# Sirui-Xu/InterDiff

Measured on AMD Instinct MI355X. Metric: denoising frame-steps/sec (denoising-steps/sec x B x T frames), higher is better.
Workload: dtype f32 (every contraction of the denoiser -- feed-forward block, QKV projection, self-attention, row-block contractions and the two token GEMMs: every fp32 operand as two f16 planes, 3 f16 MFMAs per product, fp32 accumulate; SMPL and everything else fp32 MFMA / VALU)

## Files before the change

### interdiff_amd/csrc/gemm.h

```cpp
#pragma once
#include "common.h"
#include "philox.h"

namespace idf_gemm {

enum { A_PLAIN = 0, A_LN = 1, A_TOKT = 2, A_TOKT_R = 3 };
constexpr bool is_tokt(int a) { return a == A_TOKT || a == A_TOKT_R; }
enum { E_BIAS = 0, E_GELU = 1, E_RESID = 2, E_HEADS = 3, E_EMBED = 4, E_HEADS_POST = 5, E_HEADS_POST_RAGGED = 6,
       E_SKEL = 7, E_SKEL_POST = 8, E_SKEL_POST_RAGGED = 9 };
constexpr bool is_skel(int epi) { return epi == E_SKEL || epi == E_SKEL_POST || epi == E_SKEL_POST_RAGGED; }
constexpr bool is_post(int epi) { return epi == E_HEADS_POST || epi == E_HEADS_POST_RAGGED || epi == E_SKEL_POST || epi == E_SKEL_POST_RAGGED; }

struct Args {
    const float *A;
    int lda, K;
    int Ka;
    const float *lnw, *lnb;
    size_t a_pstride;
    const float *W;
    const float *bias;
    float *C;
    int ldc, M, N;
    float *xn_out;
    const float *resid;
    int T;
    const int64_t *ts;
    const float *temb, *pe;
    int n_steps;
    float *post_x;
    const float *post_gt;
    const uint8_t *post_mask;
    const float *post_table;
    const int64_t *post_state;
#ifdef IDF_GEMM_PROBE
    long long *probe;
#endif
};

__device__ __forceinline__ void xcd_tile(int ntn, int &mt, int &nt, int &wg) {
    const int nwg = gridDim.x, id = blockIdx.x, q = nwg >> 3, r = nwg & 7, xcd = id & 7;
    wg = (xcd < r ? xcd * (q + 1) : r * (q + 1) + (xcd - r) * q) + (id >> 3);
    mt = wg / ntn;
    nt = wg - mt * ntn;
}

__device__ __forceinline__ float4 ld4(const float *p) { return *reinterpret_cast<const float4 *>(p); }
__device__ __forceinline__ float4 zero4() { return make_float4(0.f, 0.f, 0.f, 0.f); }

#ifdef IDF_GEMM_PROBE
#define IDF_PROBE_STAMP(g, wg, slot) do { if ((g).probe && threadIdx.x == 0) (g).probe[(wg) * 4 + (slot)] = clock64(); } while (0)
#else
#define IDF_PROBE_STAMP(g, wg, slot) do { } while (0)
#endif

#define IDF_MFMA4(acc, a, b)                                            \
    do {                                                                \
        acc = __builtin_amdgcn_mfma_f32_16x16x4f32(a, b, acc, 0, 0, 0); \
    } while (0)


template <int TN>
__device__ __forceinline__ void load_bias(const Args &g, float (&bv)[TN], int col0) {
#pragma unroll
    for (int j = 0; j < TN; ++j) bv[j] = g.bias ? g.bias[min(col0 + j * 16, g.N - 1)] : 0.f;
}

template <int TM, int TN>
__device__ __forceinline__ void load_resid(const Args &g, float (&rres)[TM][TN][4], int rbase0, int col0) {
#pragma unroll
    for (int i = 0; i < TM; ++i)
#pragma unroll
        for (int j = 0; j < TN; ++j) {
            const int col = min(col0 + j * 16, g.N - 1);
#pragma unroll
            for (int r = 0; r < 4; ++r) rres[i][j][r] = g.resid[(size_t)min(rbase0 + i * 16 + r, g.M - 1) * g.ldc + col];
        }
}

template <int TM, int TN>
__device__ __forceinline__ void load_embed_add(const Args &g, float (&rres)[TM][TN][4], int rbase0, int col0) {
#pragma unroll
    for (int i = 0; i < TM; ++i)
#pragma unroll
        for (int r = 0; r < 4; ++r) {
            const int rc = min(rbase0 + i * 16 + r, g.M - 1), b = rc / g.T, t = rc - b * g.T;
            int64_t step = g.ts[b];
            step = step < 0 ? 0 : (step >= g.n_steps ? g.n_steps - 1 : step);
#pragma unroll
            for (int j = 0; j < TN; ++j) {
                const int cc = min(col0 + j * 16, g.N - 1);
                rres[i][j][r] = g.temb[(size_t)step * g.N + cc] + g.pe[(size_t)t * g.N + cc];
            }
        }
}

template <int TM, int TN>
struct PostOperands {
    float4 xv[TM][TN], gv[TM][TN], e[TM][TN];
    uchar4 mk[TM][TN];
    float c1, c2, sigma;
};
__device__ __forceinline__ float sel8(const float4 a, const float4 b, int k) {
    const float lo = k == 0 ? a.x : (k == 1 ? a.y : (k == 2 ? a.z : a.w));
    const float hi = k == 4 ? b.x : (k == 5 ? b.y : (k == 6 ? b.z : b.w));
    return k < 4 ? lo : hi;
}
template <int TM, int TN, bool ragged>
__device__ __forceinline__ void post_prefetch(const Args &g, PostOperands<TM, TN> &po, int rbase0, int col0) {
    const int64_t st = g.post_state[4];
    const uint64_t it = (uint64_t)g.post_state[5], seed = (uint64_t)g.post_state[2];
    const size_t elem0 = (size_t)g.post_state[6];
    po.c1 = g.post_table[st * 4]; po.c2 = g.post_table[st * 4 + 1]; po.sigma = g.post_table[st * 4 + 2];
#pragma unroll
    for (int i = 0; i < TM; ++i)
#pragma unroll
        for (int j = 0; j < TN; ++j) {
            const int col = min(col0 + j * 16, g.N - 1);
            if constexpr (!ragged) {
                const int rbase = min(rbase0 + i * 16, g.M - 4);
                const int b = rbase / g.T, t = rbase - b * g.T;
                const size_t flat = ((size_t)b * g.N + col) * g.T + t;
                po.xv[i][j] = ld4(g.post_x + flat);
                po.gv[i][j] = g.post_mask ? ld4(g.post_gt + flat) : zero4();
                po.mk[i][j] = g.post_mask ? *reinterpret_cast<const uchar4 *>(g.post_mask + flat) : make_uchar4(0, 0, 0, 0);
                po.e[i][j] = randn4(seed, it, (uint64_t)((flat + elem0) >> 2));
            } else {
                const int r0 = min(rbase0 + i * 16, g.M - 1), b0 = r0 / g.T;
                const size_t idx0 = ((size_t)b0 * g.N + col) * g.T + (r0 - b0 * g.T) + elem0;
                const float4 ea = randn4(seed, it, (uint64_t)(idx0 >> 2)), eb = randn4(seed, it, (uint64_t)(idx0 >> 2) + 1);
                float xr[4], gr[4], er[4];
                unsigned char mr[4];
#pragma unroll
                for (int r = 0; r < 4; ++r) {
                    const int row = min(rbase0 + i * 16 + r, g.M - 1), b = row / g.T;
                    const size_t flat = ((size_t)b * g.N + col) * g.T + (row - b * g.T);
                    xr[r] = g.post_x[flat];
                    gr[r] = g.post_mask ? g.post_gt[flat] : 0.f;
                    mr[r] = g.post_mask ? g.post_mask[flat] : (unsigned char)0;
                    if (b == b0) er[r] = sel8(ea, eb, (int)(idx0 & 3) + (row - r0));
                    else {
                        const size_t idx = flat + elem0;
                        const float4 ec = randn4(seed, it, (uint64_t)(idx >> 2));
                        er[r] = sel8(ec, ec, (int)(idx & 3));
                    }
                }
                po.xv[i][j] = make_float4(xr[0], xr[1], xr[2], xr[3]);
                po.gv[i][j] = make_float4(gr[0], gr[1], gr[2], gr[3]);
                po.mk[i][j] = make_uchar4(mr[0], mr[1], mr[2], mr[3]);
                po.e[i][j] = make_float4(er[0], er[1], er[2], er[3]);
            }
            asm volatile("" : "+v"(po.e[i][j].x), "+v"(po.e[i][j].y), "+v"(po.e[i][j].z), "+v"(po.e[i][j].w));
        }
}
template <int TM, int TN, bool ragged>
__device__ __forceinline__ void epilogue_post(const Args &g, const f32x4 (&acc)[TM][TN], const float (&bvs)[TN], const PostOperands<TM, TN> &po,
                                              int rbase0, int col0, float *lds_tile = nullptr, int lds_stride = 0) {
#pragma unroll
    for (int i = 0; i < TM; ++i)
#pragma unroll
        for (int j = 0; j < TN; ++j) {
            const int rbase = rbase0 + i * 16, col = col0 + j * 16;
            if (col >= g.N || rbase >= g.M) continue;
            const float bv = bvs[j];
            float4 pv = make_float4(acc[i][j][0] + bv, acc[i][j][1] + bv, acc[i][j][2] + bv, acc[i][j][3] + bv);
            const uchar4 m = po.mk[i][j];
            const float4 gv = po.gv[i][j];
            pv.x = m.x ? gv.x : pv.x; pv.y = m.y ? gv.y : pv.y; pv.z = m.z ? gv.z : pv.z; pv.w = m.w ? gv.w : pv.w;
            const float4 out = posterior4(po.c1, po.c2, po.sigma, pv, po.xv[i][j], po.e[i][j]);
            if (lds_tile) {
                lds_tile[0] = out.x; lds_tile[lds_stride] = out.y; lds_tile[2 * lds_stride] = out.z; lds_tile[3 * lds_stride] = out.w;
            }
            if constexpr (!ragged) {
                const int b = rbase / g.T, t = rbase - b * g.T;
                idf_store16_wt(g.post_x + ((size_t)b * g.N + col) * g.T + t, out);
            } else {
                const float ov[4] = {out.x, out.y, out.z, out.w};
#pragma unroll
                for (int r = 0; r < 4; ++r) {
                    const int row = rbase + r, b = row / g.T;
                    if (row < g.M) idf_store4_wt(g.post_x + ((size_t)b * g.N + col) * g.T + (row - b * g.T), ov[r]);
                }
            }
        }
}

template <int TM, int TN, int EPI>
__device__ __forceinline__ void epilogue(const Args &g, const f32x4 (&acc)[TM][TN], const float (&rres)[TM][TN][4],
                                         const float (&bvs)[TN], int rbase0, int col0) {
    const int M = g.M, N = g.N;
#pragma unroll
    for (int i = 0; i < TM; ++i) {
        const int rbase = rbase0 + i * 16;
#pragma unroll
        for (int j = 0; j < TN; ++j) {
            const int col = col0 + j * 16;
            const bool colok = col < N;
            const float bv = bvs[j];
            if constexpr (EPI == E_HEADS) {
                if (!colok) continue;
                const int b = rbase / g.T, t = rbase - b * g.T;
                if ((g.T & 3) == 0 && rbase + 3 < M) {
                    *reinterpret_cast<float4 *>(g.C + ((size_t)b * N + col) * g.T + t) =
                        make_float4(acc[i][j][0] + bv, acc[i][j][1] + bv, acc[i][j][2] + bv, acc[i][j][3] + bv);
                } else {
#pragma unroll
                    for (int r = 0; r < 4; ++r) {
                        const int row = rbase + r;
                        if (row >= M) continue;
                        const int bb = row / g.T, tt = row - bb * g.T;
                        g.C[((size_t)bb * N + col) * g.T + tt] = acc[i][j][r] + bv;
                    }
                }
            } else {
#pragma unroll
                for (int r = 0; r < 4; ++r) {
                    const int row = rbase + r;
                    float v = acc[i][j][r] + bv;
                    if constexpr (EPI == E_GELU) v = gelu_fast(v);
                    if constexpr (EPI == E_RESID) v += rres[i][j][r];
                    if constexpr (EPI == E_EMBED) {
                        const int rc = min(row, M - 1), b = rc / g.T, t = rc - b * g.T, cc = min(col, N - 1);
                        int64_t step = g.ts[b];
                        step = step < 0 ? 0 : (step >= g.n_steps ? g.n_steps - 1 : step);
                        v += g.temb[(size_t)step * N + cc] + g.pe[(size_t)t * N + cc];
                    }
                    if (row < M && colok) g.C[(size_t)row * g.ldc + col] = v;
                }
            }
        }
    }
}

template <int BM, int BN, int TM, int TN, int EPI, int NT>
__device__ __forceinline__ void epilogue_rows(const Args &g, float *cs, const f32x4 (&acc)[TM][TN], const float (&rres)[TM][TN][4],
                                              const float (&bvs)[TN], bool writer, int wrow0, int wcol0, int kq, int li, int m0, int n0,
                                              int tid) {
    constexpr int CS = BN + 4, Q = BN / 4;
    if (writer) {
#pragma unroll
        for (int i = 0; i < TM; ++i)
#pragma unroll
            for (int j = 0; j < TN; ++j)
#pragma unroll
                for (int r = 0; r < 4; ++r) {
                    float v = acc[i][j][r] + bvs[j];
                    if constexpr (EPI == E_GELU) v = gelu_fast(v);
                    if constexpr (EPI == E_RESID || EPI == E_EMBED) v += rres[i][j][r];
                    cs[(wrow0 + i * 16 + kq * 4 + r) * CS + wcol0 + j * 16 + li] = v;
                }
    }
    __syncthreads();
    for (int idx = tid; idx < BM * Q; idx += NT) {
        const int row = idx / Q, c4 = idx - row * Q, gr = m0 + row, gc = n0 + c4 * 4;
        if (gr < g.M && gc < g.N) idf_store16_wt(g.C + (size_t)gr * g.ldc + gc, ld4(cs + row * CS + c4 * 4));
    }
}

}
#include "skel_head.h"
namespace idf_gemm {

template <int BM, int BN, int WM, int WN, int KC, int APRO, int EPI, int NP = 1>
__global__ __launch_bounds__(WM *WN * 64) void gemm_kernel(const Args g) {
    constexpr int NT = WM * WN * 64;
    constexpr int TM = BM / WM / 16, TN = BN / WN / 16;
    constexpr int QC = KC / 4;
    constexpr int AQ = BM * 4 + 4, BQ = BN * 4 + 4;
    constexpr int KLN = 256;
    constexpr int A_FLOATS = APRO == A_LN ? (KLN / 4) * AQ : 2 * QC * AQ;
    constexpr int LA = (BM * QC + NT - 1) / NT, LB = (BN * QC + NT - 1) / NT;
    static_assert(TM >= 1 && TN >= 1 && QC % 4 == 0, "tile shape");
    __shared__ __attribute__((aligned(16))) float smem[A_FLOATS + 2 * QC * BQ];
    float *As = smem, *Bs = smem + A_FLOATS;

    idf_args_now(g.A, g.lda, g.K, g.lnw, g.lnb, g.a_pstride, g.W, g.bias, g.C, g.ldc, g.M, g.N, g.xn_out, g.resid, g.T, g.ts, g.temb, g.pe, g.n_steps,
                 g.post_x, g.post_gt, g.post_mask, g.post_table, g.post_state, gridDim.x);
    const int tid = threadIdx.x, lane = tid & 63, wave = tid >> 6;
    int mt_, nt_, wg;
    xcd_tile((g.N + BN - 1) / BN, mt_, nt_, wg);
    const int m0 = mt_ * BM, n0 = nt_ * BN;
    const int wm = wave / WN, wn = wave % WN;
    const int li = lane & 15, kq = lane >> 4;
    const int K = g.K, M = g.M, N = g.N;
    const int nk = (K + KC - 1) / KC;

    float4 areg[LA], breg[LB];
    auto load_b = [&](int kc) {
#pragma unroll
        for (int i = 0; i < LB; ++i) {
            const int f = tid + NT * i;
            if ((BN * QC) % NT == 0 || f < BN * QC) {
                const int col = f / QC, q = f % QC, n = n0 + col, k = kc * KC + q * 4;
                breg[i] = (n < N && k < K) ? ld4(g.W + (size_t)n * K + k) : zero4();
            }
        }
    };
    auto store_b = [&](int buf) {
#pragma unroll
        for (int i = 0; i < LB; ++i) {
            const int f = tid + NT * i;
            if ((BN * QC) % NT == 0 || f < BN * QC) {
                const int col = f / QC, q = f % QC;
                *reinterpret_cast<float4 *>(Bs + (buf * QC + q) * BQ + col * 4) = breg[i];
            }
        }
    };
    auto load_a = [&](int kc) {
#pragma unroll
        for (int i = 0; i < LA; ++i) {
            const int f = tid + NT * i;
            if ((BM * QC) % NT == 0 || f < BM * QC) {
                if constexpr (APRO == A_TOKT) {
                    const int row = f % BM, q = f / BM, m = m0 + row, k = kc * KC + q * 4;
                    float4 v = zero4();
                    if (m < M && k < K) {
                        const int b = m / g.T, t = m - b * g.T;
                        const float *p = g.A + ((size_t)b * K + k) * g.T + t;
                        v.x = p[0];
                        v.y = p[(size_t)g.T];
                        v.z = p[(size_t)2 * g.T];
                        v.w = p[(size_t)3 * g.T];
                    }
                    areg[i] = v;
                } else if constexpr (APRO == A_TOKT_R) {
                    const int row = f % BM, q = f / BM, m = m0 + row, k = kc * KC + q * 4, Ka = g.Ka;
                    float4 v = zero4();
                    if (m < M && k < Ka) {
                        const int b = m / g.T, t = m - b * g.T;
                        const float *p = g.A + ((size_t)b * Ka + k) * g.T + t;
                        const float y = p[(size_t)min(1, Ka - 1 - k) * g.T], z = p[(size_t)min(2, Ka - 1 - k) * g.T], w_ = p[(size_t)min(3, Ka - 1 - k) * g.T];
                        v.x = p[0];
                        v.y = k + 1 < Ka ? y : 0.f;
                        v.z = k + 2 < Ka ? z : 0.f;
                        v.w = k + 3 < Ka ? w_ : 0.f;
                    }
                    areg[i] = v;
                } else {
                    const int row = f / QC, q = f % QC, m = m0 + row, k = kc * KC + q * 4;
                    areg[i] = (m < M && k < K) ? ld4(g.A + (size_t)m * g.lda + k) : zero4();
                }
            }
        }
    };
    auto store_a = [&](int buf) {
#pragma unroll
        for (int i = 0; i < LA; ++i) {
            const int f = tid + NT * i;
            if ((BM * QC) % NT == 0 || f < BM * QC) {
                const int row = is_tokt(APRO) ? f % BM : f / QC, q = is_tokt(APRO) ? f / BM : f % QC;
                *reinterpret_cast<float4 *>(As + (buf * QC + q) * AQ + row * 4) = areg[i];
            }
        }
    };

    IDF_PROBE_STAMP(g, wg, 0);
    load_b(0);
    float rres[TM][TN][4], bvs[TN];
    load_bias<TN>(g, bvs, n0 + wn * TN * 16 + li);
    if constexpr (EPI == E_RESID) load_resid<TM, TN>(g, rres, m0 + wm * TM * 16 + kq * 4, n0 + wn * TN * 16 + li);
    if constexpr (EPI == E_EMBED) load_embed_add<TM, TN>(g, rres, m0 + wm * TM * 16 + kq * 4, n0 + wn * TN * 16 + li);
    if constexpr (APRO == A_LN) {
        constexpr int NW = WM * WN;
        const float4 gw = g.lnw ? ld4(g.lnw + lane * 4) : make_float4(1.f, 1.f, 1.f, 1.f);
        const float4 gb = g.lnw ? ld4(g.lnb + lane * 4) : zero4();
#pragma unroll
        for (int i = 0; i < BM / NW; ++i) {
            const int row = wave + NW * i, m = m0 + row;
            float4 v = ld4_sum<NP>(g.A + (size_t)min(m, M - 1) * g.lda + lane * 4, g.a_pstride);
            if (g.lnw) {
                float mean, rstd;
                ln_row_stats(v, mean, rstd);
                v.x = (v.x - mean) * rstd * gw.x + gb.x;
                v.y = (v.y - mean) * rstd * gw.y + gb.y;
                v.z = (v.z - mean) * rstd * gw.z + gb.z;
                v.w = (v.w - mean) * rstd * gw.w + gb.w;
            }
            *reinterpret_cast<float4 *>(As + lane * AQ + row * 4) = v;
            if (g.xn_out && nt_ == 0 && m < M) *reinterpret_cast<float4 *>(g.xn_out + (size_t)m * KLN + lane * 4) = v;
        }
    } else {
        load_a(0);
        store_a(0);
    }
    store_b(0);
    __syncthreads();
    IDF_PROBE_STAMP(g, wg, 1);

    f32x4 acc[TM][TN];
#pragma unroll
    for (int i = 0; i < TM; ++i)
#pragma unroll
        for (int j = 0; j < TN; ++j) acc[i][j] = f32x4{0.f, 0.f, 0.f, 0.f};

    for (int kc = 0; kc < nk; ++kc) {
        const int buf = kc & 1;
        if (kc + 1 < nk) {
            load_b(kc + 1);
            if constexpr (APRO != A_LN) load_a(kc + 1);
        }
        const float *Ab = APRO == A_LN ? As + kc * QC * AQ : As + buf * QC * AQ;
        const float *Bb = Bs + buf * QC * BQ;
#pragma unroll
        for (int s = 0; s < QC / 4; ++s) {
            float4 a[TM], b[TN];
#pragma unroll
            for (int i = 0; i < TM; ++i) a[i] = ld4(Ab + (s * 4 + kq) * AQ + ((wm * TM + i) * 16 + li) * 4);
#pragma unroll
            for (int j = 0; j < TN; ++j) b[j] = ld4(Bb + (s * 4 + kq) * BQ + ((wn * TN + j) * 16 + li) * 4);
#pragma unroll
            for (int i = 0; i < TM; ++i)
#pragma unroll
                for (int j = 0; j < TN; ++j) IDF_MFMA4(acc[i][j], a[i].x, b[j].x);
#pragma unroll
            for (int i = 0; i < TM; ++i)
#pragma unroll
                for (int j = 0; j < TN; ++j) IDF_MFMA4(acc[i][j], a[i].y, b[j].y);
#pragma unroll
            for (int i = 0; i < TM; ++i)
#pragma unroll
                for (int j = 0; j < TN; ++j) IDF_MFMA4(acc[i][j], a[i].z, b[j].z);
#pragma unroll
            for (int i = 0; i < TM; ++i)
#pragma unroll
                for (int j = 0; j < TN; ++j) IDF_MFMA4(acc[i][j], a[i].w, b[j].w);
        }
        if (kc + 1 < nk) {
            store_b(buf ^ 1);
            if constexpr (APRO != A_LN) store_a(buf ^ 1);
        }
        __syncthreads();
    }

    IDF_PROBE_STAMP(g, wg, 2);
    if constexpr (EPI == E_BIAS || EPI == E_GELU || EPI == E_RESID || EPI == E_EMBED) {
        static_assert(BM * (BN + 4) <= A_FLOATS + 2 * QC * BQ, "C tile must fit the operand buffers");
        epilogue_rows<BM, BN, TM, TN, EPI, NT>(g, smem, acc, rres, bvs, true, wm * TM * 16, wn * TN * 16, kq, li, m0, n0, tid);
    } else {
        epilogue<TM, TN, EPI>(g, acc, rres, bvs, m0 + wm * TM * 16 + kq * 4, n0 + wn * TN * 16 + li);
    }
    IDF_PROBE_STAMP(g, wg, 3);
}

template <int BM, int BN, int WM, int WN, int KC, int APRO, int EPI, int NP = 1>
inline void launch(hipStream_t s, const Args &g) {
    dim3 grid((unsigned)(idf_cdiv(g.M, BM) * idf_cdiv(g.N, BN)));
    hipLaunchKernelGGL((gemm_kernel<BM, BN, WM, WN, KC, APRO, EPI, NP>), grid, dim3(WM * WN * 64), 0, s, g);
}

template <int N>
__device__ __forceinline__ void wait_vmcnt() {
    static_assert(N >= 0 && N <= 16, "vmcnt literal");
#define IDF_VMCNT_CASE(n) if constexpr (N == n) asm volatile("s_waitcnt vmcnt(" #n ")" ::: "memory");
    IDF_VMCNT_CASE(0) IDF_VMCNT_CASE(1) IDF_VMCNT_CASE(2) IDF_VMCNT_CASE(3) IDF_VMCNT_CASE(4) IDF_VMCNT_CASE(5) IDF_VMCNT_CASE(6)
    IDF_VMCNT_CASE(7) IDF_VMCNT_CASE(8) IDF_VMCNT_CASE(9) IDF_VMCNT_CASE(10) IDF_VMCNT_CASE(11) IDF_VMCNT_CASE(12)
    IDF_VMCNT_CASE(13) IDF_VMCNT_CASE(14) IDF_VMCNT_CASE(15) IDF_VMCNT_CASE(16)
#undef IDF_VMCNT_CASE
}

template <int BM, int BN, int WM, int WN, int KS, int KC, int APRO, int EPI, int NS = 3, int NP = 1>
__global__ __launch_bounds__(WM *WN *KS * 64) void gemm_glds_kernel(const Args g) {
    constexpr int NWT = WM * WN, NW = NWT * KS;
    constexpr int TM = BM / WM / 16, TN = BN / WN / 16;
    constexpr int CH = KC / 4;
    constexpr int RSL = 256 + 4;
    constexpr int A_STAGE = APRO == A_LN ? 0 : BM * KC, STAGE = A_STAGE + BN * KC;
    constexpr int A_LN_FLOATS = APRO == A_LN ? BM * RSL : 0;
    constexpr int IA = A_STAGE / 256, IB = BN * KC / 256, IPC = IA + IB, LPC = IPC / NW;
    constexpr int RED = KS > 1 ? (KS - 1) * NWT * 64 * TM * TN * 4 : 0;
    static_assert(IPC % NW == 0 && LPC >= 1 && (NS - 2) * LPC <= 16 && NS >= 3 && NS <= 6, "chunk loads must split evenly over the waves");
    static_assert((CH / 4) % KS == 0 && TM >= 1 && TN >= 1 && (CH == 8 || CH == 16), "tile shape");
    static_assert(APRO != A_TOKT, "token gather uses the register-staged kernel");
    constexpr int SMEM = A_LN_FLOATS + NS * STAGE;
    __shared__ __attribute__((aligned(1024))) float smem[SMEM > RED ? SMEM : RED];
    float *Aln = smem, *stages = smem + A_LN_FLOATS;

    idf_args_now(g.A, g.lda, g.K, g.lnw, g.lnb, g.a_pstride, g.W, g.bias, g.C, g.ldc, g.M, g.N, g.xn_out, g.resid, g.T, g.ts, g.temb, g.pe, g.n_steps,
                 g.post_x, g.post_gt, g.post_mask, g.post_table, g.post_state, gridDim.x);
    const int tid = threadIdx.x, lane = tid & 63;
    const int wave = __builtin_amdgcn_readfirstlane(tid >> 6);
    int mt_, nt_, wg;
    xcd_tile((g.N + BN - 1) / BN, mt_, nt_, wg);
    const int m0 = mt_ * BM, n0 = nt_ * BN;
    const int ks = wave / NWT, wt = wave % NWT, wm = wt / WN, wn = wt % WN;
    const int li = lane & 15, kq = lane >> 4;
    const int K = g.K, M = g.M, N = g.N;
    const int nk = K / KC;
    IDF_PROBE_STAMP(g, wg, 0);

    const float *src[LPC];
    int dst[LPC];
#pragma unroll
    for (int j = 0; j < LPC; ++j) {
        const int i = wave + NW * j;
        if (i < IA) {
            const int p = i * 64 + lane, row = p / CH, c = (p % CH) ^ (row % CH);
            src[j] = g.A + (size_t)min(m0 + row, M - 1) * g.lda + c * 4;
            dst[j] = i * 256;
        } else {
            const int ib = i - IA, p = ib * 64 + lane, row = p / CH, c = (p % CH) ^ (row % CH);
            src[j] = g.W + (size_t)min(n0 + row, N - 1) * K + c * 4;
            dst[j] = A_STAGE + ib * 256;
        }
    }
    auto wait_landed = [&](int c) {
        const int ahead = min(NS - 2, nk - 1 - c);
        if (ahead <= 0) wait_vmcnt<0>();
        else if (ahead == 1) wait_vmcnt<LPC>();
        else if (ahead == 2) { if constexpr (NS >= 4) wait_vmcnt<2 * LPC>(); }
        else if (ahead == 3) { if constexpr (NS >= 5) wait_vmcnt<3 * LPC>(); }
        else { if constexpr (NS >= 6) wait_vmcnt<4 * LPC>(); }
    };
    const uint32_t stages_lds = idf_lds_addr(stages);
    auto issue = [&](int kc, int st) {
#pragma unroll
        for (int j = 0; j < LPC; ++j) idf_dma16_v(src[j] + kc * KC, stages_lds + (uint32_t)((st * STAGE + dst[j]) * 4));
    };

#pragma unroll
    for (int c = 0; c < NS - 1; ++c)
        if (c < nk) issue(c, c);
    float rres[TM][TN][4], bvs[TN];
    load_bias<TN>(g, bvs, n0 + wn * TN * 16 + li);
    if constexpr (EPI == E_RESID) {
        if (ks == 0) load_resid<TM, TN>(g, rres, m0 + wm * TM * 16 + kq * 4, n0 + wn * TN * 16 + li);
    }
    PostOperands<is_post(EPI) && !is_skel(EPI) ? TM : 1, is_post(EPI) && !is_skel(EPI) ? TN : 1> po;
    SkelPre skp;
    if constexpr (is_skel(EPI)) {
        static_assert(!is_skel(EPI) || (BM == 32 && BN == 32 && NW == 8 && SMEM >= 32 * SKH_CS + 32 * SKH_ZMAX), "the keypoint head's tile: 32 x 32, 512 threads");
        skel_prefetch<EPI>(g, skp, m0, nt_, tid);
    } else if constexpr (is_post(EPI)) {
        if (ks == 0) post_prefetch<TM, TN, EPI == E_HEADS_POST_RAGGED>(g, po, m0 + wm * TM * 16 + kq * 4, n0 + wn * TN * 16 + li);
    }
    if constexpr (APRO == A_LN) {
        const float4 gw = g.lnw ? ld4(g.lnw + lane * 4) : make_float4(1.f, 1.f, 1.f, 1.f);
        const float4 gb = g.lnw ? ld4(g.lnb + lane * 4) : zero4();
#pragma unroll
        for (int i = 0; i < BM / NW; ++i) {
            const int row = wave + NW * i, m = m0 + row;
            float4 v = ld4_sum<NP>(g.A + (size_t)min(m, M - 1) * g.lda + lane * 4, g.a_pstride);
            if (g.lnw) {
                float mean, rstd;
                ln_row_stats(v, mean, rstd);
                v.x = (v.x - mean) * rstd * gw.x + gb.x;
                v.y = (v.y - mean) * rstd * gw.y + gb.y;
                v.z = (v.z - mean) * rstd * gw.z + gb.z;
                v.w = (v.w - mean) * rstd * gw.w + gb.w;
            }
            *reinterpret_cast<float4 *>(Aln + row * RSL + lane * 4) = v;
            if (g.xn_out && nt_ == 0 && m < M) *reinterpret_cast<float4 *>(g.xn_out + (size_t)m * 256 + lane * 4) = v;
        }
    }
    wait_landed(0);
    __builtin_amdgcn_s_waitcnt(0xc07f);
    __builtin_amdgcn_s_barrier();
    IDF_PROBE_STAMP(g, wg, 1);

    f32x4 acc[TM][TN];
#pragma unroll
    for (int i = 0; i < TM; ++i)
#pragma unroll
        for (int j = 0; j < TN; ++j) acc[i][j] = f32x4{0.f, 0.f, 0.f, 0.f};

    int aoff[TM], akey[TM], boff[TN], bkey[TN];
#pragma unroll
    for (int i = 0; i < TM; ++i) {
        const int row = (wm * TM + i) * 16 + li;
        aoff[i] = APRO == A_LN ? row * RSL : row * KC;
        akey[i] = row % CH;
    }
#pragma unroll
    for (int j = 0; j < TN; ++j) {
        const int row = (wn * TN + j) * 16 + li;
        boff[j] = row * KC;
        bkey[j] = row % CH;
    }

    int st = 0;
    for (int kc = 0; kc < nk; ++kc) {
        if (kc + NS - 1 < nk) issue(kc + NS - 1, st >= 1 ? st - 1 : NS - 1);
        const float *Ab = APRO == A_LN ? Aln + kc * KC : stages + st * STAGE;
        const float *Bb = stages + st * STAGE + A_STAGE;
#pragma unroll
        for (int s2 = 0; s2 < CH / 4 / KS; ++s2) {
            const int c = (s2 * KS + ks) * 4 + kq;
            float4 a[TM], b[TN];
#pragma unroll
            for (int i = 0; i < TM; ++i) a[i] = ld4(Ab + aoff[i] + (APRO == A_LN ? c : (c ^ akey[i])) * 4);
#pragma unroll
            for (int j = 0; j < TN; ++j) b[j] = ld4(Bb + boff[j] + (c ^ bkey[j]) * 4);
#pragma unroll
            for (int i = 0; i < TM; ++i)
#pragma unroll
                for (int j = 0; j < TN; ++j) IDF_MFMA4(acc[i][j], a[i].x, b[j].x);
#pragma unroll
            for (int i = 0; i < TM; ++i)
#pragma unroll
                for (int j = 0; j < TN; ++j) IDF_MFMA4(acc[i][j], a[i].y, b[j].y);
#pragma unroll
            for (int i = 0; i < TM; ++i)
#pragma unroll
                for (int j = 0; j < TN; ++j) IDF_MFMA4(acc[i][j], a[i].z, b[j].z);
#pragma unroll
            for (int i = 0; i < TM; ++i)
#pragma unroll
                for (int j = 0; j < TN; ++j) IDF_MFMA4(acc[i][j], a[i].w, b[j].w);
        }
        wait_landed(kc + 1);
        __builtin_amdgcn_s_waitcnt(0xc07f);
        __builtin_amdgcn_s_barrier();
        st = st == NS - 1 ? 0 : st + 1;
    }
    IDF_PROBE_STAMP(g, wg, 2);

    if constexpr (KS > 1) {
        constexpr int SLAB = NWT * 64 * TM * TN * 4;
        float *red = smem + (size_t)(wt * 64 + lane) * (TM * TN * 4);
        if (ks > 0) {
#pragma unroll
            for (int i = 0; i < TM; ++i)
#pragma unroll
                for (int j = 0; j < TN; ++j) *reinterpret_cast<f32x4 *>(red + (ks - 1) * SLAB + (i * TN + j) * 4) = acc[i][j];
        }
        __syncthreads();
        if (ks == 0) {
#pragma unroll
            for (int q = 0; q < KS - 1; ++q)
#pragma unroll
                for (int i = 0; i < TM; ++i)
#pragma unroll
                    for (int j = 0; j < TN; ++j) acc[i][j] += *reinterpret_cast<const f32x4 *>(red + q * SLAB + (i * TN + j) * 4);
        }
    }
    if constexpr (EPI == E_BIAS || EPI == E_GELU || EPI == E_RESID) {
        static_assert(BM * (BN + 4) <= (SMEM > RED ? SMEM : RED), "C tile must fit the operand buffers");
        if constexpr (KS > 1) __syncthreads();
        epilogue_rows<BM, BN, TM, TN, EPI, NW * 64>(g, smem, acc, rres, bvs, ks == 0, wm * TM * 16, wn * TN * 16, kq, li, m0, n0, tid);
    } else if constexpr (is_skel(EPI)) {
        __syncthreads();
        if (ks == 0) {
#pragma unroll
            for (int i = 0; i < TM; ++i)
#pragma unroll
                for (int j = 0; j < TN; ++j)
#pragma unroll
                    for (int r = 0; r < 4; ++r) smem[((wm * TM + i) * 16 + kq * 4 + r) * SKH_CS + (wn * TN + j) * 16 + li] = acc[i][j][r] + bvs[j];
        }
        skel_epilogue<EPI>(g, smem, smem + 32 * SKH_CS, skp, m0, nt_, tid);
    } else {
        if constexpr (is_post(EPI)) {
            if (ks == 0) epilogue_post<TM, TN, EPI == E_HEADS_POST_RAGGED>(g, acc, bvs, po, m0 + wm * TM * 16 + kq * 4, n0 + wn * TN * 16 + li);
        } else {
            if (ks == 0) epilogue<TM, TN, EPI>(g, acc, rres, bvs, m0 + wm * TM * 16 + kq * 4, n0 + wn * TN * 16 + li);
        }
    }
    IDF_PROBE_STAMP(g, wg, 3);
}

template <int BM, int BN, int WM, int WN, int KS, int KC, int APRO, int EPI, int NS = 3, int NP = 1>
inline void launch_glds(hipStream_t s, const Args &g) {
    dim3 grid((unsigned)(idf_cdiv(g.M, BM) * idf_cdiv(g.N, BN)));
    hipLaunchKernelGGL((gemm_glds_kernel<BM, BN, WM, WN, KS, KC, APRO, EPI, NS, NP>), grid, dim3(WM * WN * KS * 64), 0, s, g);
}

}
```

### interdiff_amd/csrc/tail_h2.h

```cpp
#pragma once
#include "common.h"
#include "gemm.h"
#include "ffn_h2.h"

namespace idf_tail_h2 {

using idf_ffn_h2::h8;
constexpr int D = IDF_MDM_D, CW = 144, TRW = 16, NTH = 512, NWV = NTH / 64;
constexpr int NTO = CW / 16, KSH = D / 32;
constexpr int KE = 160, KSE = KE / 32, NTE = D / 16;
constexpr int OUT_H2_FLOATS = NTO * KSH * 2 * 64 * 4, IN_H2_FLOATS = NTE * KSE * 2 * 64 * 4;
constexpr int RHS = D + 8;
constexpr int XTS = CW + 4;
constexpr int XHS = KE + 8;
constexpr int USS = D + 4;

struct TailArgs {
    const float *u_in;
    size_t pstride;
    const float *ln_w, *ln_b;
    const float *wout, *out_b;
    float *x0;
    idf_gemm::Args post;
    const float *x_tok;
    const float *win, *in_b, *temb, *pe;
    const int64_t *ts;
    int n_steps;
    float *u0;
    int M, T;
    int plain_ids;
};

template <int MODE, bool RAGGED>
__global__ __launch_bounds__(NTH) void step_tail_h2_kernel(const float *__restrict__ u_in, size_t u_pstride, const float *__restrict__ wout, int M, int T, int nwg,
                                                           int plain_ids, const TailArgs a) {
    constexpr bool HEADS = MODE != 0, EMBED = MODE == 0 || MODE == 3, POST = MODE >= 2;
    asm volatile("" ::: "v255");
    __shared__ __attribute__((aligned(16))) _Float16 rpl[HEADS ? 2 * TRW * RHS : 8];
    __shared__ __attribute__((aligned(16))) float xt[EMBED ? TRW * XTS : 4];
    __shared__ __attribute__((aligned(16))) _Float16 xpl[EMBED ? 2 * TRW * XHS : 8];
    __shared__ float sc[TRW];
    __shared__ __attribute__((aligned(16))) float us[EMBED ? TRW * USS : 4];
    const int tid = threadIdx.x, lane = tid & 63, wave = tid >> 6, li = lane & 15, kq = lane >> 4;
    const int wid = blockIdx.x, xq = nwg >> 3, xr = nwg & 7, xcd = wid & 7;
    const int tile = plain_ids ? wid : (xcd < xr ? xcd * (xq + 1) : xr * (xq + 1) + (xcd - xr) * xq) + (wid >> 3);
    const int m0 = tile * TRW;
    const int rown = (wave & 3) * 4 + kq;
    const bool rowpass = wave < 4;

    if constexpr (HEADS) {
        constexpr int NTW = 2;
        const int ntw = wave == 0 ? 2 : 1;
        auto tile_of = [&](int j) { return j == 0 ? wave : NTO - 1; };
        Row16Raw<IDF_FFN_SLICES> raw;
        if (rowpass) raw.request(u_in + (size_t)min(m0 + rown, M - 1) * D, li, u_pstride);
        idf_gemm::PostOperands<1, 1> po[NTW];
        if constexpr (POST) {
#pragma unroll
            for (int j = 0; j < NTW; ++j)
                if (j < ntw) idf_gemm::post_prefetch<1, 1, RAGGED>(a.post, po[j], m0 + kq * 4, tile_of(j) * 16 + li);
        }
        float4 wf[NTW][KSH][2];
#pragma unroll
        for (int j = 0; j < NTW; ++j)
            if (j < ntw) {
#pragma unroll
                for (int s = 0; s < KSH; ++s)
#pragma unroll
                    for (int pl = 0; pl < 2; ++pl) wf[j][s][pl] = idf_gemm::ld4(wout + (size_t)(((tile_of(j) * KSH + s) * 2 + pl) * 64 + lane) * 4);
            }
        if (rowpass) {
            Row16 r;
            raw.reduce(r);
            ln_row16(r, a.ln_w, a.ln_b, li);
            idf_ffn_h2::row16_store_planes(r, rpl + rown * RHS, rpl + (TRW + rown) * RHS, li);
        }
        __syncthreads();
        f32x4 am[NTW], ac[NTW];
#pragma unroll
        for (int j = 0; j < NTW; ++j) am[j] = ac[j] = f32x4{0.f, 0.f, 0.f, 0.f};
        h8 ah[KSH], al[KSH];
#pragma unroll
        for (int s = 0; s < KSH; ++s) {
            ah[s] = *reinterpret_cast<const h8 *>(rpl + li * RHS + 32 * s + 8 * kq);
            al[s] = *reinterpret_cast<const h8 *>(rpl + (TRW + li) * RHS + 32 * s + 8 * kq);
        }
#pragma unroll
        for (int j = 0; j < NTW; ++j)
            if (j < ntw) {
#pragma unroll
                for (int s = 0; s < KSH; ++s) {
                    IDF_H2_MFMA(am[j], ah[s], __builtin_bit_cast(h8, wf[j][s][0]));
                    IDF_H2_MFMA(ac[j], ah[s], __builtin_bit_cast(h8, wf[j][s][1]));
                    IDF_H2_MFMA(ac[j], al[s], __builtin_bit_cast(h8, wf[j][s][0]));
                }
            }
#pragma unroll
        for (int j = 0; j < NTW; ++j)
            if (j < ntw) {
                const int col = tile_of(j) * 16 + li, rbase = m0 + kq * 4;
                const float bv = a.out_b[col];
                f32x4 v;
#pragma unroll
                for (int q = 0; q < 4; ++q) v[q] = am[j][q] + ac[j][q] * idf_ffn_h2::LO_UNSCALE;
                if constexpr (POST) {
                    const f32x4 accs[1][1] = {{v}};
                    const float bvs[1] = {bv};
                    idf_gemm::epilogue_post<1, 1, RAGGED>(a.post, accs, bvs, po[j], rbase, col, EMBED ? xt + (kq * 4) * XTS + col : nullptr, XTS);
                } else {
                    if (!RAGGED && rbase + 3 < M) {
                        const int b = rbase / T, t = rbase - b * T;
                        *reinterpret_cast<float4 *>(a.x0 + ((size_t)b * CW + col) * T + t) = make_float4(v[0] + bv, v[1] + bv, v[2] + bv, v[3] + bv);
                    } else {
#pragma unroll
                        for (int q = 0; q < 4; ++q) {
                            const int row = rbase + q;
                            if (row < M) {
                                const int bb = row / T;
                                a.x0[((size_t)bb * CW + col) * T + (row - bb * T)] = v[q] + bv;
                            }
                        }
                    }
                }
            }
    }

    if constexpr (EMBED) {
        if constexpr (MODE == 0) {
            if constexpr (!RAGGED) {
#pragma unroll
                for (int it = 0; it < (CW * 4 + NTH - 1) / NTH; ++it) {
                    const int idx = tid + it * NTH, c = min(idx >> 2, CW - 1), rg = idx & 3;
                    const int rowb = min(m0 + 4 * rg, M - 4), b = rowb / T, t = rowb - b * T;
                    const float4 v = idf_gemm::ld4(a.x_tok + ((size_t)b * CW + c) * T + t);
                    if (idx < CW * 4) {
                        float *d = xt + (4 * rg) * XTS + c;
                        d[0] = v.x; d[XTS] = v.y; d[2 * XTS] = v.z; d[3 * XTS] = v.w;
                    }
                }
            } else {
#pragma unroll
                for (int it = 0; it < (CW * TRW + NTH - 1) / NTH; ++it) {
                    const int idx = tid + it * NTH, c = min(idx >> 4, CW - 1), rl = idx & 15, row = min(m0 + rl, M - 1), b = row / T;
                    const float v = a.x_tok[((size_t)b * CW + c) * T + (row - b * T)];
                    if (idx < CW * TRW) xt[rl * XTS + c] = v;
                }
            }
        }
        constexpr int NTEW = NTE / NWV;
        float4 ef[NTEW][KSE][2];
#pragma unroll
        for (int j = 0; j < NTEW; ++j)
#pragma unroll
            for (int s = 0; s < KSE; ++s)
#pragma unroll
                for (int pl = 0; pl < 2; ++pl) ef[j][s][pl] = idf_gemm::ld4(a.win + (size_t)((((wave * NTEW + j) * KSE + s) * 2 + pl) * 64 + lane) * 4);
        constexpr int NST = TRW * (D / 4) / NTH;
        float4 eb[NST], et[NST], ep[NST];
#pragma unroll
        for (int it = 0; it < NST; ++it) {
            const int idx = tid + it * NTH, rl = idx >> 6, c4 = (idx & 63) << 2, row = min(m0 + rl, M - 1), b = row / T, t = row - b * T;
            int64_t step = a.ts[b];
            step = step < 0 ? 0 : (step >= a.n_steps ? a.n_steps - 1 : step);
            eb[it] = idf_gemm::ld4(a.in_b + c4);
            et[it] = idf_gemm::ld4(a.temb + (size_t)step * D + c4);
            ep[it] = idf_gemm::ld4(a.pe + (size_t)t * D + c4);
        }
        __syncthreads();
        if (rowpass) {
            float4 c[3];
#pragma unroll
            for (int k = 0; k < 3; ++k) c[k] = li + 16 * k < CW / 4 ? *reinterpret_cast<const float4 *>(xt + rown * XTS + 4 * (li + 16 * k)) : make_float4(0.f, 0.f, 0.f, 0.f);
            float amax = 0.f;
#pragma unroll
            for (int k = 0; k < 3; ++k) amax = fmaxf(amax, fmaxf(fmaxf(__builtin_fabsf(c[k].x), __builtin_fabsf(c[k].y)), fmaxf(__builtin_fabsf(c[k].z), __builtin_fabsf(c[k].w))));
            amax = row16_max(amax);
            const int e = (amax > 0.f && amax < INFINITY) ? (int)((__builtin_bit_cast(uint32_t, amax) >> 23) & 0xff) - 126 : 0;
            const float dn = __builtin_bit_cast(float, (uint32_t)((127 - e) << 23)), up = __builtin_bit_cast(float, (uint32_t)((127 + e) << 23));
            _Float16 *xh = xpl + rown * XHS, *xl = xpl + (TRW + rown) * XHS;
#pragma unroll
            for (int k = 0; k < 3; ++k) {
                const int ch = li + 16 * k;
                if (ch < KE / 4) {
                    uint2 h, l;
                    idf_ffn_h2::split4_pk(make_float4(c[k].x * dn, c[k].y * dn, c[k].z * dn, c[k].w * dn), h, l);
                    *reinterpret_cast<uint2 *>(xh + 4 * ch) = h;
                    *reinterpret_cast<uint2 *>(xl + 4 * ch) = l;
                }
            }
            if (li == 0) sc[rown] = up;
        }
        __syncthreads();
        f32x4 em[NTEW], ec[NTEW];
#pragma unroll
        for (int j = 0; j < NTEW; ++j) em[j] = ec[j] = f32x4{0.f, 0.f, 0.f, 0.f};
#pragma unroll
        for (int s = 0; s < KSE; ++s) {
            const h8 ah = *reinterpret_cast<const h8 *>(xpl + li * XHS + 32 * s + 8 * kq), al = *reinterpret_cast<const h8 *>(xpl + (TRW + li) * XHS + 32 * s + 8 * kq);
#pragma unroll
            for (int j = 0; j < NTEW; ++j) {
                IDF_H2_MFMA(em[j], ah, __builtin_bit_cast(h8, ef[j][s][0]));
                IDF_H2_MFMA(ec[j], ah, __builtin_bit_cast(h8, ef[j][s][1]));
                IDF_H2_MFMA(ec[j], al, __builtin_bit_cast(h8, ef[j][s][0]));
            }
        }
#pragma unroll
        for (int j = 0; j < NTEW; ++j)
#pragma unroll
            for (int q = 0; q < 4; ++q) us[(kq * 4 + q) * USS + (wave * NTEW + j) * 16 + li] = (em[j][q] + ec[j][q] * idf_ffn_h2::LO_UNSCALE) * sc[kq * 4 + q];
        __syncthreads();
#pragma unroll
        for (int it = 0; it < NST; ++it) {
            const int idx = tid + it * NTH, rl = idx >> 6, c4 = (idx & 63) << 2;
            float4 v = *reinterpret_cast<const float4 *>(us + rl * USS + c4);
            v.x += eb[it].x; v.y += eb[it].y; v.z += eb[it].z; v.w += eb[it].w;
            v.x += et[it].x + ep[it].x; v.y += et[it].y + ep[it].y; v.z += et[it].z + ep[it].z; v.w += et[it].w + ep[it].w;
            if (m0 + rl < M) idf_store16_wt(a.u0 + (size_t)(m0 + rl) * D + c4, v);
        }
    }
}

template <int MODE, bool RAGGED>
inline int launch_tail_one(hipStream_t s, const TailArgs *ta) {
    static idf_excl_cache excl;
    static const char *const names[4] = {"step_tail_h2_kernel<embed>", "step_tail_h2_kernel<heads>", "step_tail_h2_kernel<heads+update>", "step_tail_h2_kernel<heads+update+embed>"};
    const int dyn = idf_exclusive_cu(reinterpret_cast<const void *>(&step_tail_h2_kernel<MODE, RAGGED>), names[MODE], NTH, excl);
    if (!ta) return dyn;
    if (dyn < 0) return IDF_NOT_EXCLUSIVE;
    hipLaunchKernelGGL((step_tail_h2_kernel<MODE, RAGGED>), dim3((unsigned)idf_cdiv(ta->M, TRW)), dim3(NTH), (size_t)dyn, s, ta->u_in, ta->pstride, ta->wout, ta->M, ta->T,
                       (int)idf_cdiv(ta->M, TRW), ta->plain_ids, *ta);
    return IDF_OK;
}
inline int launch_tail_sel(hipStream_t s, int mode, bool ragged, const TailArgs *ta) {
    switch (mode * 2 + (ragged ? 1 : 0)) {
    case 0: return launch_tail_one<0, false>(s, ta);
    case 1: return launch_tail_one<0, true>(s, ta);
    case 2: return launch_tail_one<1, false>(s, ta);
    case 3: return launch_tail_one<1, true>(s, ta);
    case 4: return launch_tail_one<2, false>(s, ta);
    case 5: return launch_tail_one<2, true>(s, ta);
    case 6: return launch_tail_one<3, false>(s, ta);
    default: return launch_tail_one<3, true>(s, ta);
    }
}
inline int launch_tail(hipStream_t s, int mode, const TailArgs &ta) { return launch_tail_sel(s, mode, (ta.T & 3) != 0, &ta); }
inline bool tail_exclusive_ok(bool ragged) {
    bool ok = true;
    for (int mode = 0; mode < 4; ++mode) ok = (launch_tail_sel(nullptr, mode, ragged, nullptr) >= 0) && ok;
    return ok;
}

}
```

Baseline: 6.996 million.

## Reschedule tail kernel loads to overlap posterior and embedding prefetch with MFMA

Splits the posterior prefetch into scalar, operand and noise phases so the fused tail kernel can schedule each separately. In mode 3 the row-pass waves defer their posterior operand/noise loads and the next-block embedding weight and bias loads until after the output-head MFMAs, using sched barriers, so that load latency overlaps compute and register pressure before the MFMAs drops. It also moves the second output-weight tile load to wave 4 and after the layernorm, hoists bias loads, and makes the per-row embedding indices wave-uniform. The risk is that deferred loads now sit on the critical path after the MFMAs, and the extra live registers may reduce occupancy.

Result: no change. 6.991 million (median of 2 runs) (-0.1%).

```diff
diff --git a/interdiff_amd/csrc/gemm.h b/interdiff_amd/csrc/gemm.h
--- a/interdiff_amd/csrc/gemm.h
+++ b/interdiff_amd/csrc/gemm.h
@@ -105,12 +105,18 @@
     const float hi = k == 4 ? b.x : (k == 5 ? b.y : (k == 6 ? b.z : b.w));
     return k < 4 ? lo : hi;
 }
+struct PostKeys {
+    uint64_t it, seed;
+    size_t elem0;
+};
+template <int TM, int TN>
+__device__ __forceinline__ PostKeys post_prefetch_scalars(const Args &g, PostOperands<TM, TN> &po) {
+    const int64_t st = g.post_state[4];
+    po.c1 = g.post_table[st * 4]; po.c2 = g.post_table[st * 4 + 1]; po.sigma = g.post_table[st * 4 + 2];
+    return PostKeys{(uint64_t)g.post_state[5], (uint64_t)g.post_state[2], (size_t)g.post_state[6]};
+}
 template <int TM, int TN, bool ragged>
-__device__ __forceinline__ void post_prefetch(const Args &g, PostOperands<TM, TN> &po, int rbase0, int col0) {
-    const int64_t st = g.post_state[4];
-    const uint64_t it = (uint64_t)g.post_state[5], seed = (uint64_t)g.post_state[2];
-    const size_t elem0 = (size_t)g.post_state[6];
-    po.c1 = g.post_table[st * 4]; po.c2 = g.post_table[st * 4 + 1]; po.sigma = g.post_table[st * 4 + 2];
+__device__ __forceinline__ void post_prefetch_operands(const Args &g, PostOperands<TM, TN> &po, int rbase0, int col0) {
 #pragma unroll
     for (int i = 0; i < TM; ++i)
 #pragma unroll
@@ -123,12 +129,8 @@
                 po.xv[i][j] = ld4(g.post_x + flat);
                 po.gv[i][j] = g.post_mask ? ld4(g.post_gt + flat) : zero4();
                 po.mk[i][j] = g.post_mask ? *reinterpret_cast<const uchar4 *>(g.post_mask + flat) : make_uchar4(0, 0, 0, 0);
-                po.e[i][j] = randn4(seed, it, (uint64_t)((flat + elem0) >> 2));
             } else {
-                const int r0 = min(rbase0 + i * 16, g.M - 1), b0 = r0 / g.T;
-                const size_t idx0 = ((size_t)b0 * g.N + col) * g.T + (r0 - b0 * g.T) + elem0;
-                const float4 ea = randn4(seed, it, (uint64_t)(idx0 >> 2)), eb = randn4(seed, it, (uint64_t)(idx0 >> 2) + 1);
-                float xr[4], gr[4], er[4];
+                float xr[4], gr[4];
                 unsigned char mr[4];
 #pragma unroll
                 for (int r = 0; r < 4; ++r) {
@@ -137,20 +139,52 @@
                     xr[r] = g.post_x[flat];
                     gr[r] = g.post_mask ? g.post_gt[flat] : 0.f;
                     mr[r] = g.post_mask ? g.post_mask[flat] : (unsigned char)0;
+                }
+                po.xv[i][j] = make_float4(xr[0], xr[1], xr[2], xr[3]);
+                po.gv[i][j] = make_float4(gr[0], gr[1], gr[2], gr[3]);
+                po.mk[i][j] = make_uchar4(mr[0], mr[1], mr[2], mr[3]);
+            }
+        }
+}
+template <int TM, int TN, bool ragged>
+__device__ __forceinline__ void post_prefetch_noise(const Args &g, const PostKeys &k, PostOperands<TM, TN> &po, int rbase0, int col0) {
+    const uint64_t it = k.it, seed = k.seed;
+    const size_t elem0 = k.elem0;
+#pragma unroll
+    for (int i = 0; i < TM; ++i)
+#pragma unroll
+        for (int j = 0; j < TN; ++j) {
+            const int col = min(col0 + j * 16, g.N - 1);
+            if constexpr (!ragged) {
+                const int rbase = min(rbase0 + i * 16, g.M - 4);
+                const int b = rbase / g.T, t = rbase - b * g.T;
+                const size_t flat = ((size_t)b * g.N + col) * g.T + t;
+                po.e[i][j] = randn4(seed, it, (uint64_t)((flat + elem0) >> 2));
+            } else {
+                const int r0 = min(rbase0 + i * 16, g.M - 1), b0 = r0 / g.T;
+                const size_t idx0 = ((size_t)b0 * g.N + col) * g.T + (r0 - b0 * g.T) + elem0;
+                const float4 ea = randn4(seed, it, (uint64_t)(idx0 >> 2)), eb = randn4(seed, it, (uint64_t)(idx0 >> 2) + 1);
+                float er[4];
+#pragma unroll
+                for (int r = 0; r < 4; ++r) {
+                    const int row = min(rbase0 + i * 16 + r, g.M - 1), b = row / g.T;
                     if (b == b0) er[r] = sel8(ea, eb, (int)(idx0 & 3) + (row - r0));
                     else {
-                        const size_t idx = flat + elem0;
+                        const size_t idx = ((size_t)b * g.N + col) * g.T + (row - b * g.T) + elem0;
                         const float4 ec = randn4(seed, it, (uint64_t)(idx >> 2));
                         er[r] = sel8(ec, ec, (int)(idx & 3));
                     }
                 }
-                po.xv[i][j] = make_float4(xr[0], xr[1], xr[2], xr[3]);
-                po.gv[i][j] = make_float4(gr[0], gr[1], gr[2], gr[3]);
-                po.mk[i][j] = make_uchar4(mr[0], mr[1], mr[2], mr[3]);
                 po.e[i][j] = make_float4(er[0], er[1], er[2], er[3]);
             }
             asm volatile("" : "+v"(po.e[i][j].x), "+v"(po.e[i][j].y), "+v"(po.e[i][j].z), "+v"(po.e[i][j].w));
         }
+}
+template <int TM, int TN, bool ragged>
+__device__ __forceinline__ void post_prefetch(const Args &g, PostOperands<TM, TN> &po, int rbase0, int col0) {
+    const PostKeys k = post_prefetch_scalars(g, po);
+    post_prefetch_operands<TM, TN, ragged>(g, po, rbase0, col0);
+    post_prefetch_noise<TM, TN, ragged>(g, k, po, rbase0, col0);
 }
 template <int TM, int TN, bool ragged>
 __device__ __forceinline__ void epilogue_post(const Args &g, const f32x4 (&acc)[TM][TN], const float (&bvs)[TN], const PostOperands<TM, TN> &po,
diff --git a/interdiff_amd/csrc/tail_h2.h b/interdiff_amd/csrc/tail_h2.h
--- a/interdiff_amd/csrc/tail_h2.h
+++ b/interdiff_amd/csrc/tail_h2.h
@@ -48,33 +48,84 @@
     const int rown = (wave & 3) * 4 + kq;
     const bool rowpass = wave < 4;
 
+    constexpr int NTEW = NTE / NWV;
+    constexpr int NST = TRW * (D / 4) / NTH;
+    float4 ef[NTEW][KSE][2], eb[NST], et[NST], ep[NST];
+    int64_t estep[NST];
+    int eframe[NST];
+    const int wave_s = __builtin_amdgcn_readfirstlane(wave);
+    [[maybe_unused]] auto embed_rows = [&]() {
+#pragma unroll
+        for (int it = 0; it < NST; ++it) {
+            const int row = min(m0 + wave_s + it * (NTH / 64), M - 1), b = row / T;
+            const int64_t step = a.ts[b];
+            estep[it] = step < 0 ? 0 : (step >= a.n_steps ? a.n_steps - 1 : step);
+            eframe[it] = row - b * T;
+        }
+    };
+    [[maybe_unused]] auto request_embed = [&]() {
+#pragma unroll
+        for (int j = 0; j < NTEW; ++j)
+#pragma unroll
+            for (int s = 0; s < KSE; ++s)
+#pragma unroll
+                for (int pl = 0; pl < 2; ++pl) ef[j][s][pl] = idf_gemm::ld4(a.win + (size_t)((((wave * NTEW + j) * KSE + s) * 2 + pl) * 64 + lane) * 4);
+#pragma unroll
+        for (int it = 0; it < NST; ++it) {
+            const int c4 = lane << 2;
+            eb[it] = idf_gemm::ld4(a.in_b + c4);
+            et[it] = idf_gemm::ld4(a.temb + (size_t)estep[it] * D + c4);
+            ep[it] = idf_gemm::ld4(a.pe + (size_t)eframe[it] * D + c4);
+        }
+    };
+
     if constexpr (HEADS) {
         constexpr int NTW = 2;
-        const int ntw = wave == 0 ? 2 : 1;
+        constexpr bool DEFER = MODE == 3;
+        const int ntw = wave == 4 ? 2 : 1;
         auto tile_of = [&](int j) { return j == 0 ? wave : NTO - 1; };
         Row16Raw<IDF_FFN_SLICES> raw;
         if (rowpass) raw.request(u_in + (size_t)min(m0 + rown, M - 1) * D, li, u_pstride);
+        if constexpr (MODE == 3) embed_rows();
         idf_gemm::PostOperands<1, 1> po[NTW];
+        idf_gemm::PostKeys pk{};
+        float bvj[NTW];
+#pragma unroll
+        for (int j = 0; j < NTW; ++j)
+            if (j < ntw) bvj[j] = a.out_b[tile_of(j) * 16 + li];
         if constexpr (POST) {
+            pk = idf_gemm::post_prefetch_scalars(a.post, po[0]);
+            if constexpr (DEFER) {
+                auto uni = [](uint64_t v) {
+                    return (uint64_t)(uint32_t)__builtin_amdgcn_readfirstlane((int)(uint32_t)v) | ((uint64_t)(uint32_t)__builtin_amdgcn_readfirstlane((int)(uint32_t)(v >> 32)) << 32);
+                };
+                pk.it = uni(pk.it); pk.seed = uni(pk.seed); pk.elem0 = (size_t)uni((uint64_t)pk.elem0);
+            }
 #pragma unroll
             for (int j = 0; j < NTW; ++j)
-                if (j < ntw) idf_gemm::post_prefetch<1, 1, RAGGED>(a.post, po[j], m0 + kq * 4, tile_of(j) * 16 + li);
+                if (j < ntw) {
+                    po[j].c1 = po[0].c1; po[j].c2 = po[0].c2; po[j].sigma = po[0].sigma;
+                    if (!(DEFER && rowpass)) {
+                        idf_gemm::post_prefetch_operands<1, 1, RAGGED>(a.post, po[j], m0 + kq * 4, tile_of(j) * 16 + li);
+                        idf_gemm::post_prefetch_noise<1, 1, RAGGED>(a.post, pk, po[j], m0 + kq * 4, tile_of(j) * 16 + li);
+                    }
+                }
         }
         float4 wf[NTW][KSH][2];
-#pragma unroll
-        for (int j = 0; j < NTW; ++j)
-            if (j < ntw) {
-#pragma unroll
-                for (int s = 0; s < KSH; ++s)
-#pragma unroll
-                    for (int pl = 0; pl < 2; ++pl) wf[j][s][pl] = idf_gemm::ld4(wout + (size_t)(((tile_of(j) * KSH + s) * 2 + pl) * 64 + lane) * 4);
-            }
+        auto request_wf = [&](int j) {
+#pragma unroll
+            for (int s = 0; s < KSH; ++s)
+#pragma unroll
+                for (int pl = 0; pl < 2; ++pl) wf[j][s][pl] = idf_gemm::ld4(wout + (size_t)(((tile_of(j) * KSH + s) * 2 + pl) * 64 + lane) * 4);
+        };
+        request_wf(0);
         if (rowpass) {
             Row16 r;
             raw.reduce(r);
             ln_row16(r, a.ln_w, a.ln_b, li);
             idf_ffn_h2::row16_store_planes(r, rpl + rown * RHS, rpl + (TRW + rown) * RHS, li);
         }
+        if (ntw > 1) request_wf(1);
         __syncthreads();
         f32x4 am[NTW], ac[NTW];
 #pragma unroll
@@ -95,11 +146,19 @@
                     IDF_H2_MFMA(ac[j], al[s], __builtin_bit_cast(h8, wf[j][s][0]));
                 }
             }
+        if constexpr (MODE == 3) {
+            __builtin_amdgcn_sched_barrier(0);
+            if (rowpass) idf_gemm::post_prefetch_operands<1, 1, RAGGED>(a.post, po[0], m0 + kq * 4, tile_of(0) * 16 + li);
+            request_embed();
+            __builtin_amdgcn_sched_barrier(0);
+        }
+        if constexpr (POST && DEFER)
+            if (rowpass) idf_gemm::post_prefetch_noise<1, 1, RAGGED>(a.post, pk, po[0], m0 + kq * 4, tile_of(0) * 16 + li);
 #pragma unroll
         for (int j = 0; j < NTW; ++j)
             if (j < ntw) {
                 const int col = tile_of(j) * 16 + li, rbase = m0 + kq * 4;
-                const float bv = a.out_b[col];
+                const float bv = bvj[j];
                 f32x4 v;
 #pragma unroll
                 for (int q = 0; q < 4; ++q) v[q] = am[j][q] + ac[j][q] * idf_ffn_h2::LO_UNSCALE;
@@ -146,25 +205,8 @@
                     if (idx < CW * TRW) xt[rl * XTS + c] = v;
                 }
             }
-        }
-        constexpr int NTEW = NTE / NWV;
-        float4 ef[NTEW][KSE][2];
-#pragma unroll
-        for (int j = 0; j < NTEW; ++j)
-#pragma unroll
-            for (int s = 0; s < KSE; ++s)
-#pragma unroll
-                for (int pl = 0; pl < 2; ++pl) ef[j][s][pl] = idf_gemm::ld4(a.win + (size_t)((((wave * NTEW + j) * KSE + s) * 2 + pl) * 64 + lane) * 4);
-        constexpr int NST = TRW * (D / 4) / NTH;
-        float4 eb[NST], et[NST], ep[NST];
-#pragma unroll
-        for (int it = 0; it < NST; ++it) {
-            const int idx = tid + it * NTH, rl = idx >> 6, c4 = (idx & 63) << 2, row = min(m0 + rl, M - 1), b = row / T, t = row - b * T;
-            int64_t step = a.ts[b];
-            step = step < 0 ? 0 : (step >= a.n_steps ? a.n_steps - 1 : step);
-            eb[it] = idf_gemm::ld4(a.in_b + c4);
-            et[it] = idf_gemm::ld4(a.temb + (size_t)step * D + c4);
-            ep[it] = idf_gemm::ld4(a.pe + (size_t)t * D + c4);
+            embed_rows();
+            request_embed();
         }
         __syncthreads();
         if (rowpass) {
```
